# NVlabs/CenterPose

Measured on NVIDIA H100. Metric: images/sec at 512x512 DLA-34 (dla_34 + DCNv2, 7 heads, decode + PnP), higher is better.
Workload: dtype tf32x3

## Files before the change

### centerpose_b200/_lib.py

```python
import ctypes
import os

HERE = os.path.dirname(os.path.abspath(__file__))
LIB_PATH = os.environ.get("CP_LIB_PATH") or os.path.join(HERE, "libcenterpose_b200.so")

CP_MAX_HEADS = 16
CP_POSE_RECORD = 192
CP_DETS_RECORD = 128
CP_META_DOUBLES = 16
CP_MAX_K = 128
CP_MAX_MODELS = 16

CP_ARCH_DLA34 = 0
CP_ARCH_DLAV1_34 = 1
CP_ARCH_RES_18, CP_ARCH_RES_34, CP_ARCH_RES_50, CP_ARCH_RES_101, CP_ARCH_RES_152 = 2, 3, 4, 5, 6
CP_PREC_FP32 = 0
CP_PREC_TF32X3 = 1
CP_PREC_BF16 = 2
CP_PREC_TF32 = 3
PRECISIONS = {"fp32": CP_PREC_FP32, "tf32x3": CP_PREC_TF32X3, "bf16": CP_PREC_BF16, "tf32": CP_PREC_TF32}

P_SCORE, P_CLS, P_STATUS, P_NPTS, P_BBOX, P_CT, P_KPS = 0, 1, 2, 3, 4, 8, 10
P_KPS_DISP_MEAN, P_KPS_HM_MEAN, P_KPS_HM_STD, P_KPS_HM_HEIGHT, P_KPS_DISP_STD = 26, 42, 58, 74, 82
P_OBJ_SCALE, P_OBJ_SCALE_UNC, P_TRACKING, P_TRACKING_HP = 98, 101, 104, 106
# ... 39 lines not shown
FAM_NONE, FAM_IGEMM_FP32, FAM_STEM, FAM_CONV3_C16, FAM_IGEMM_UMMA, FAM_CONV_TMA, FAM_DCN_TMA = 0, 1, 2, 3, 4, 5, 6
FAM_MAXPOOL, FAM_UPADD, FAM_GN_RELU, FAM_GRU = 7, 8, 9, 10
FAMILY_NAMES = {FAM_NONE: "fused", FAM_IGEMM_FP32: "igemm_fp32", FAM_STEM: "stem", FAM_CONV3_C16: "conv3_c16",
                FAM_IGEMM_UMMA: "igemm_umma", FAM_CONV_TMA: "conv_tma", FAM_DCN_TMA: "dcn_tma", FAM_MAXPOOL: "maxpool",
                FAM_UPADD: "upadd", FAM_GN_RELU: "gn_relu", FAM_GRU: "gru"}


class CpOpStat(ctypes.Structure):
    _fields_ = [("name", ctypes.c_char * 96), ("kind", ctypes.c_int32), ("ms", ctypes.c_float),
                ("flops", ctypes.c_double), ("bytes", ctypes.c_double)]


class CpActDesc(ctypes.Structure):
    _fields_ = [("off", ctypes.c_int64), ("ext", ctypes.c_int32), ("C", ctypes.c_int32), ("H", ctypes.c_int32),
                ("W", ctypes.c_int32), ("stride", ctypes.c_int32)]


class CpOpDesc(ctypes.Structure):
    _fields_ = ([("name", ctypes.c_char * 96)] +
                [(n, ctypes.c_int32) for n in ("kind", "family", "x3", "nsrc")] +
                [("src", CpActDesc * 4), ("out", CpActDesc), ("out_head", ctypes.c_int32)] +
                [(n, ctypes.c_int32) for n in ("kh", "stride", "pad", "Cin", "Cout", "CoutPad", "Kpad")] +
                [("w", ctypes.c_void_p), ("w_ld", ctypes.c_int32), ("bias", ctypes.c_void_p)] +
                [(n, ctypes.c_int32) for n in ("relu", "has_res", "res_after_relu")] +
                [("res", CpActDesc), ("om", CpActDesc), ("up_w", ctypes.c_void_p), ("f", ctypes.c_int32),
                 ("has_skip", ctypes.c_int32), ("skip", CpActDesc), ("gamma", ctypes.c_void_p),
                 ("beta", ctypes.c_void_p), ("groups", ctypes.c_int32), ("gx", CpActDesc), ("gh", CpActDesc),
                 ("gprev", CpActDesc), ("first_step", ctypes.c_int32)] +
                [(n, ctypes.c_int32) for n in ("fuse_heads", "fused_away", "parent", "n_children")] +
                [("children", ctypes.c_int32 * CP_MAX_HEADS)])


class CpOpLaunch(ctypes.Structure):
    _fields_ = [(n, ctypes.c_int32) for n in ("family", "BN", "ksplit", "grid")]


class CpMemoryInfo(ctypes.Structure):
    _fields_ = [(n, ctypes.c_int64) for n in ("activation_bytes", "weight_bytes", "tile_bytes", "workspace_bytes")]


class CpActAlloc(ctypes.Structure):
    _fields_ = [("floats", ctypes.c_int64), ("off", ctypes.c_int64), ("first", ctypes.c_int32), ("last", ctypes.c_int32)]


class CpConfig(ctypes.Structure):
    _fields_ = [
        ("arch", ctypes.c_int32), ("tracking", ctypes.c_int32), ("tracking_task_gru", ctypes.c_int32),
        ("max_batch", ctypes.c_int32), ("height", ctypes.c_int32), ("width", ctypes.c_int32),
        ("precision", ctypes.c_int32), ("device", ctypes.c_int32), ("head_conv", ctypes.c_int32),
        ("num_heads", ctypes.c_int32),
        ("head_names", ctypes.c_char_p * CP_MAX_HEADS),
        ("head_channels", ctypes.c_int32 * CP_MAX_HEADS),
    ]


class CpHeads(ctypes.Structure):
    _fields_ = [(n, ctypes.c_void_p) for n in (
        "hm", "wh", "hps", "reg", "hm_hp", "hp_offset", "scale", "hps_uncertainty",
        "scale_uncertainty", "tracking", "tracking_hp")]


class CpDecodeParams(ctypes.Structure):
    _fields_ = [
        ("batch", ctypes.c_int32), ("out_h", ctypes.c_int32), ("out_w", ctypes.c_int32),
        ("num_classes", ctypes.c_int32), ("num_joints", ctypes.c_int32), ("K", ctypes.c_int32),
        ("rep_mode", ctypes.c_int32), ("use_moments", ctypes.c_int32), ("nms", ctypes.c_int32),
        ("visible_thresh", ctypes.c_int32), ("opencv_return", ctypes.c_int32),
# ... 126 lines not shown
```

### centerpose_b200/csrc/common.cuh

```cuda
#pragma once
#include <cuda_runtime.h>
#include <stdint.h>
#include <stdio.h>
#include <string>

#include "../../include/centerpose_b200.h"

namespace cp {

void set_error(const std::string& msg);
int fail(int code, const std::string& msg);
extern thread_local long long g_launch_counter;

#define CP_CUDA_CHECK(expr)                                                              \
  do {                                                                                   \
    cudaError_t _e = (expr);                                                             \
    if (_e != cudaSuccess)                                                               \
      return ::cp::fail(CP_ERR_CUDA, std::string(#expr) + ": " + cudaGetErrorString(_e)); \
  } while (0)

#define CP_LAUNCH_CHECK(what)                                                            \
  do {                                                                                   \
    cudaError_t _e = cudaGetLastError();                                                 \
    if (_e != cudaSuccess)                                                               \
// ... 25 lines not shown
  int resStride;
  int relu;
  int res_after_relu;
  float* out;
  int outStride;
  int out_nchw;
  const float* offmask;
  int omStride;
  int mask_is_logit;
  int mode;
  const void* wgt_umma;
  float* splitk_ws;
  size_t splitk_ws_floats;
  int fuse_n, fuse_hidden;
  const float* fuse_w[16];
  const float* fuse_b[16];
  float* fuse_out[16];
  int fuse_cout[16];
  int ipm;
  long long wstride, tstride;
  unsigned nchw_per_model;
};
inline int model_ipm(const IgemmParams& p) { return p.ipm > 0 ? p.ipm : p.B; }

int launch_igemm_fp32(const IgemmParams& p, cudaStream_t stream);

int decode_pnp_models(const cp_decode_params* prm, int models, const cp_heads* heads, const double* meta, float* dets,
                      float* poses, int32_t* n_valid, void* workspace, size_t workspace_bytes, void* stream);

struct LaunchInfo {
  int BN = 0;
  int ksplit = 1;
  long long grid = 0;
};

bool conv3_c16_supported(const IgemmParams& p);
int launch_conv3_c16(const IgemmParams& p, cudaStream_t stream);
bool stem_supported(const IgemmParams& p);
int launch_stem_conv(const IgemmParams& p, cudaStream_t s);

struct ConvKernel {
  int family = CP_FAM_IGEMM_FP32;
  bool x3 = false;
  bool round_out = false;
  int BN = 0;
  int cslab = 0;
  size_t wbytes = 0;
};
struct ConvPolicy {
  bool small_on_cuda_cores;
  bool dcn_tma;
  bool round_out;
  bool cuda_core_fallback;
};
inline bool known_precision(int32_t precision) {
  return precision == CP_PREC_FP32 || precision == CP_PREC_TF32X3 || precision == CP_PREC_BF16 || precision == CP_PREC_TF32;
}
inline bool gather_x3(int32_t precision) { return precision == CP_PREC_TF32 || precision == CP_PREC_TF32X3; }
ConvKernel select_conv_kernel(const IgemmParams& p, int32_t precision, const ConvPolicy& pol);
struct alignas(64) TmaMaps {
  unsigned char map[4][128];
};
int conv_encode(const ConvKernel& k, const IgemmParams& p, int Bmax, TmaMaps* maps);
int conv_pack(const ConvKernel& k, const IgemmParams& p, int ld, void* tiles, cudaStream_t s);
int conv_launch(const ConvKernel& k, const IgemmParams& p, const TmaMaps* maps, cudaStream_t s, LaunchInfo* info = nullptr);
int run_conv(IgemmParams& p, int32_t precision, const ConvPolicy& pol, cudaStream_t s);
// ... 101 lines not shown
```

### centerpose_b200/csrc/dcn_tma.cu

```cuda
#include <cuda.h>

#include "common.cuh"
#include "umma_common.cuh"

namespace cp {
namespace {

using namespace umma;

constexpr int DT_BM = 128;
constexpr int DT_THREADS = 512;
constexpr int DT_CS = 16;
constexpr int DT_PH = 8, DT_PW = 16;
constexpr int DT_HALO = 8;
constexpr int DT_SH = DT_PH + 2 * DT_HALO, DT_SW = DT_PW + 2 * DT_HALO;
constexpr uint32_t DT_SLAB_BYTES = DT_SH * DT_SW * DT_CS * 4;
constexpr uint32_t DT_COEF_BYTES = DT_BM * 9 * 16;

struct DcnTmaParams {
  CUtensorMap amap;
  const float* src;
  int srcStride;
  const float* offmask;
  int omStride, mask_is_logit;
  int B, H, W, Cin, Cout, CoutPad, BN;
  int tiles_x, tiles_per_image;
  long long total_tiles;
  int SB;
  int group;
  int AH;
  const float* bias;
  const float* residual;
  int resStride, relu, res_after_relu;
  float* out;
  int outStride, out_nchw, round_tf32;
  const unsigned char* wtiles;
  int ksplit, sps;
  float* part;
  int ipm;
  long long wstride, tstride;
};

struct DcnCtl {
  unsigned long long s_full[2], s_empty[2];
  unsigned long long a_full[2], a_empty[2];
  unsigned long long c_full[2], c_empty[2];
  unsigned long long b_full[8], b_empty[8];
};

constexpr int RB_DX = 14, RB_DY = 15, RB_W = 16, RB_SLAB = 20, RB_LIVE = 21;

__device__ __forceinline__ void coef_row(const DcnTmaParams& p, const float* __restrict__ om, int oy, int ox, int ys,
                                         int xs, uint32_t dst) {
  float o[27];
#pragma unroll
  for (int j = 0; j < 27; ++j) o[j] = __ldg(om + j);
  const int H = p.H, W = p.W;
#pragma unroll
  for (int tap = 0; tap < 9; ++tap) {
    const int ky = tap / 3, kx = tap - ky * 3;
    float mm = o[18 + tap];
    if (p.mask_is_logit) mm = 1.0f / (1.0f + expf(-mm));
    const float h_im = (float)(oy - 1 + ky) + o[2 * tap], w_im = (float)(ox - 1 + kx) + o[2 * tap + 1];
    float lh = 0.f, lw = 0.f, mk = 0.f;
    uint32_t pk = 0;
    if (h_im > -1.f && w_im > -1.f && h_im < (float)H && w_im < (float)W) {
      const int h_low = (int)floorf(h_im), w_low = (int)floorf(w_im);
      lh = h_im - (float)h_low;
      lw = w_im - (float)w_low;
      const bool t_ok = h_low >= 0, b_ok = h_low + 1 <= H - 1, l_ok = w_low >= 0, r_ok = w_low + 1 <= W - 1;
      const int hl = t_ok ? h_low : 0, hb = b_ok ? h_low + 1 : H - 1;
      const int wl = l_ok ? w_low : 0, wr = r_ok ? w_low + 1 : W - 1;
      const bool in_slab = (hl >= ys) && (hb < ys + DT_SH) && (wl >= xs) && (wr < xs + DT_SW);
      pk = in_slab ? (uint32_t)((hl - ys) * DT_SW + (wl - xs)) : (uint32_t)((hl << 7) | wl);
      pk |= (uint32_t)(wr - wl) << RB_DX;
      pk |= (uint32_t)(hb - hl) << RB_DY;
      pk |= (uint32_t)((t_ok && l_ok) ? 1 : 0) << (RB_W + 0);
      pk |= (uint32_t)((t_ok && r_ok) ? 1 : 0) << (RB_W + 1);
// ... 162 lines not shown
            }
#pragma unroll
            for (int c = 0; c < 4; ++c) {
              c3[c] = ld_shared_v4f(b3 ^ ((uint32_t)c << 4));
              c4[c] = ld_shared_v4f(b4 ^ ((uint32_t)c << 4));
            }
#pragma unroll
            for (int c = 0; c < 4; ++c) {
              v[c].x = w1 * c1[c].x + w2 * c2[c].x + w3 * c3[c].x + w4 * c4[c].x;
              v[c].y = w1 * c1[c].y + w2 * c2[c].y + w3 * c3[c].y + w4 * c4[c].y;
              v[c].z = w1 * c1[c].z + w2 * c2[c].z + w3 * c3[c].z + w4 * c4[c].z;
              v[c].w = w1 * c1[c].w + w2 * c2[c].w + w3 * c3[c].w + w4 * c4[c].w;
            }
          } else {
            const int hl = (int)((pk >> 7) & 127u), wl = (int)(pk & 127u);
            const float* g = gimg + ((size_t)hl * p.W + wl) * p.srcStride + (s0 + s) * DT_CS;
            const size_t dx = (size_t)((pk >> RB_DX) & 1u) * p.srcStride;
            const size_t dy = (size_t)((pk >> RB_DY) & 1u) * p.W * p.srcStride;
#pragma unroll
            for (int c = 0; c < 4; ++c) {
              const float4 c1 = __ldg(reinterpret_cast<const float4*>(g) + c);
              const float4 c2 = __ldg(reinterpret_cast<const float4*>(g + dx) + c);
              const float4 c3 = __ldg(reinterpret_cast<const float4*>(g + dy) + c);
              const float4 c4 = __ldg(reinterpret_cast<const float4*>(g + dy + dx) + c);
              v[c].x = w1 * c1.x + w2 * c2.x + w3 * c3.x + w4 * c4.x;
              v[c].y = w1 * c1.y + w2 * c2.y + w3 * c3.y + w4 * c4.y;
              v[c].z = w1 * c1.z + w2 * c2.z + w3 * c3.z + w4 * c4.z;
              v[c].w = w1 * c1.w + w2 * c2.w + w3 * c3.w + w4 * c4.w;
            }
          }
        }
        const int sa = (int)(cnt & (uint32_t)(p.AH - 1));
        const uint32_t a_dst = a_row + (uint32_t)sa * a_stage + (asw << 4);
        mbar_wait(smem_u32(&ctl->a_empty[sa]), ((cnt >> (p.AH - 1)) & 1u) ^ 1u);
#pragma unroll
        for (int c = 0; c < 4; ++c) {
          const uint32_t off = (uint32_t)c << 4;
          if (X3)
            st_shared_v4f(a_dst ^ off, v[c].x, v[c].y, v[c].z, v[c].w);
          else
            st_shared_v4f(a_dst ^ off, tf32_round(v[c].x), tf32_round(v[c].y), tf32_round(v[c].z), tf32_round(v[c].w));
        }
        fence_proxy_async_smem();
        __syncwarp();
        if (lane == 0) mbar_arrive(smem_u32(&ctl->a_full[sa]));
        ++cnt;
      }
      __syncwarp();
      if (lane == 0) {
        mbar_arrive(smem_u32(&ctl->s_empty[ss]));
        mbar_arrive(smem_u32(&ctl->c_empty[cb]));
      }
      if (++ss == 2) {
        ss = 0;
        ps ^= 1u;
      }
      if (++cb == 2) {
        cb = 0;
        pc ^= 1u;
      }
    }
  } else {
    asm volatile("setmaxnreg.inc.sync.aligned.u32 176;");
    const int c = warp >= 12 ? 1 : 0, wt = tid & 127;
    float* dstage = reinterpret_cast<float*>(smem + (drain0 - sbase)) + (size_t)c * (DRAIN_STAGE_BYTES / 4);
    EpiParams ep;
    ep.bias = p.bias;
// ... 2 lines not shown
    ep.relu = p.relu;
    ep.res_after_relu = p.res_after_relu;
    ep.round_tf32 = p.round_tf32;
    ep.out = p.out;
    ep.outStride = p.outStride;
    ep.out_nchw = p.out_nchw;
    ep.Cout = p.Cout;
    ep.CoutPad = p.CoutPad;
    ep.H = p.H;
    ep.W = p.W;
    int cb = 0;
    uint32_t pc = 0;
    auto make_records = [&](long long t) {
      const long long mt = (t / KS_SPLIT) / n_tiles;
      const int im = (int)(mt / p.tiles_per_image);
      const int pt = (int)(mt - (long long)im * p.tiles_per_image);
      const int y0 = (pt / p.tiles_x) * DT_PH, x0 = (pt % p.tiles_x) * DT_PW;
      const int oy = y0 + (wt >> 4), ox = x0 + (wt & 15);
      mbar_wait(smem_u32(&ctl->c_empty[cb]), pc ^ 1u);
      coef_row(p, p.offmask + ((size_t)((size_t)im * p.H + oy) * p.W + ox) * p.omStride, oy, ox, y0 - DT_HALO, x0 - DT_HALO,
               coef0 + (uint32_t)cb * DT_COEF_BYTES + (uint32_t)wt * 144u);
      __syncwarp();
      if (lane == 0) mbar_arrive(smem_u32(&ctl->c_full[cb]));
      if (++cb == 2) {
        cb = 0;
        pc ^= 1u;
      }
    };
    if (c == 0 && (long long)blockIdx.x < total_tiles) make_records(blockIdx.x);
    const uint32_t bar_a_full = smem_u32(&ctl->a_full[0]), bar_a_empty = smem_u32(&ctl->a_empty[0]);
    const uint32_t bar_b_full = smem_u32(&ctl->b_full[0]), bar_b_empty = smem_u32(&ctl->b_empty[0]);
    int sb = 0;
    uint32_t pb = 0, cnt = 0;
    float acc[BN / 2];
    float sums[X3 ? BN / 2 : 1];
#pragma unroll
    for (int j = 0; j < BN / 2; ++j) acc[j] = 0.f;
    for (long long tile = blockIdx.x; tile < total_tiles; tile += gridDim.x) {
      if (c == 0 && tile + gridDim.x < total_tiles) make_records(tile + gridDim.x);
#pragma unroll
      for (int j = 0; j < (X3 ? BN / 2 : 1); ++j) sums[j] = 0.f;
      int gk = 0;
      for (int kbi = 0; kbi < KB; ++kbi, ++cnt) {
        const uint32_t sa = cnt & (uint32_t)(p.AH - 1);
        mbar_wait(bar_a_full + 8u * sa, (cnt >> (p.AH - 1)) & 1u);
        mbar_wait(bar_b_full + 8u * (uint32_t)sb, pb);
        const uint32_t a_tile = atiles0 + sa * a_stage + (uint32_t)c * 64u * 64u;
        const uint64_t db = make_desc(btiles0 + (uint32_t)sb * btile_bytes, DT_CS);
        if (X3)
          mma_kblock_x3<BN, 2>(acc, a_tile, wt, db, ((uint32_t)BN * 64u) >> 4, gk == 0);
        else
          mma_kblock<BN, false, false, 2>(acc, make_desc(a_tile, DT_CS), db, 0, 0, kbi == 0);
        if (wt == 0) {
          mbar_arrive(bar_a_empty + 8u * sa);
          mbar_arrive(bar_b_empty + 8u * (uint32_t)sb);
        }
        if (++sb == p.SB) {
          sb = 0;
          pb ^= 1u;
        }
        if (X3) {
          if (gk == p.group - 1 || kbi == KB - 1) {
#pragma unroll
            for (int j = 0; j < (X3 ? BN / 2 : 1); ++j) sums[j] += acc[X3 ? j : 0];
            gk = 0;
          } else {
            ++gk;
          }
        }
      }
      const int n_tile = (int)((tile / KS_SPLIT) % n_tiles);
      const long long m_tile = (tile / KS_SPLIT) / n_tiles;
      const int n = (int)(m_tile / p.tiles_per_image);
      const int pt = (int)(m_tile - (long long)n * p.tiles_per_image);
      const int col_end = min(p.Cout, (n_tile + 1) * BN);
      if (MULTI) ep.bias = p.bias + (size_t)(n / p.ipm) * p.wstride;
      auto fn = [&](int r, int cb0, float (&v)[16]) {
        if (cb0 >= BN) return;
        const int i = c * 64 + r;
        if (KS_SPLIT > 1) {
          float4* part_row = reinterpret_cast<float4*>(p.part) + ((size_t)tile * (BN >> 2) + (cb0 >> 2)) * 128 + i;
#pragma unroll
          for (int q = 0; q < 4; ++q) __stcg(part_row + (size_t)q * 128, make_float4(v[4 * q], v[4 * q + 1], v[4 * q + 2], v[4 * q + 3]));
        } else {
          const int oy = (pt / p.tiles_x) * DT_PH + (i >> 4), ox = (pt % p.tiles_x) * DT_PW + (i & 15);
          const int m = (n * p.H + oy) * p.W + ox;
          epilogue_row<16>(ep, v, true, m, n, oy, ox, n_tile * BN + cb0, col_end);
        }
      };
      if constexpr (X3)
        drain_rows<BN>(sums, dstage, wt, 1 + c, fn);
      else
        drain_rows<BN>(acc, dstage, wt, 1 + c, fn);
    }
  }
}

template <bool MULTI>
__global__ void __launch_bounds__(256) dcn_tma_splitk_finish(const __grid_constant__ DcnTmaParams p, long long mn_tiles) {
  splitk_finish<MULTI>(p, DT_BM, mn_tiles, [&](long long mn, int i, int* n, int* oy, int* ox) {
    const long long m_tile = mn / (p.CoutPad / p.BN);
// ... 18 lines not shown
  return dcn_tma_tile_n(p.CoutPad, x3) != 0;
}

int dcn_tma_encode(const IgemmParams& p, int Bmax, void* map_out) {
  return tma_encode_nhwc_box(p.src[0], p.srcC[0], p.Win, p.Hin, Bmax, p.srcStride[0], DT_CS, DT_SW, DT_SH, 1, map_out);
}

int launch_dcn_tma(const IgemmParams& p, const void* map, const ConvKernel& k, cudaStream_t stream, LaunchInfo* info) {
  const bool x3 = k.x3;
  if (!p.wgt_umma) return fail(CP_ERR_INVALID, "dcn_tma: weight tiles missing");
  if (!dcn_tma_supported(p, x3)) return fail(CP_ERR_INVALID, "dcn_tma: unsupported shape");
  DcnTmaParams q;
  memset(&q, 0, sizeof(q));
  memcpy(&q.amap, map, sizeof(CUtensorMap));
  q.src = p.src[0];
  q.srcStride = p.srcStride[0];
  q.offmask = p.offmask;
  q.omStride = p.omStride;
  q.mask_is_logit = p.mask_is_logit;
  q.B = p.B;
  q.H = p.Hin;
  q.W = p.Win;
  q.Cin = p.Cin;
  q.Cout = p.Cout;
  q.CoutPad = p.CoutPad;
  q.BN = k.BN;
  q.tiles_x = p.Win / DT_PW;
  q.tiles_per_image = q.tiles_x * (p.Hin / DT_PH);
  const long long mn = (long long)q.tiles_per_image * p.B * (p.CoutPad / q.BN);
  const uint32_t a_stage = 8192u;
  q.group = kX3GroupBlocks * 2;
  const uint32_t btile = (uint32_t)q.BN * 64u * (x3 ? 2u : 1u);
  const size_t budget = 226 * 1024;
  q.AH = 2;
  size_t fixed = 1024 + 2 * (size_t)DT_COEF_BYTES + 1024 + 2 * (size_t)DT_SLAB_BYTES + (size_t)q.AH * a_stage +
                 2 * (size_t)DRAIN_STAGE_BYTES;
  if (fixed + 3 * (size_t)btile > budget) {
    q.AH = 1;
    fixed -= a_stage;
  }
  if (fixed + 2 * (size_t)btile > budget) return fail(CP_ERR_INVALID, "dcn_tma: tile does not fit shared memory");
  q.SB = (int)((budget - fixed) / btile);
  if (q.SB > 8) q.SB = 8;
  q.bias = p.bias;
  q.residual = p.residual;
  q.resStride = p.resStride;
  q.relu = p.relu;
  q.res_after_relu = p.res_after_relu;
  q.out = p.out;
  q.outStride = p.outStride;
  q.out_nchw = p.out_nchw;
  q.round_tf32 = k.round_out;
  q.wtiles = (const unsigned char*)p.wgt_umma;
  q.ipm = model_ipm(p);
  q.wstride = p.wstride;
  q.tstride = p.tstride;
  const bool multi = p.B > q.ipm;
  const size_t smem = fixed + (size_t)q.SB * btile;
  void (*kern)(DcnTmaParams) = nullptr;
  switch (q.BN) {
    case 16: kern = multi ? (x3 ? dcn_tma_kernel<true, 16, true> : dcn_tma_kernel<false, 16, true>)
                          : (x3 ? dcn_tma_kernel<true, 16, false> : dcn_tma_kernel<false, 16, false>); break;
    case 32: kern = multi ? (x3 ? dcn_tma_kernel<true, 32, true> : dcn_tma_kernel<false, 32, true>)
                          : (x3 ? dcn_tma_kernel<true, 32, false> : dcn_tma_kernel<false, 32, false>); break;
    case 64: kern = multi ? (x3 ? dcn_tma_kernel<true, 64, true> : dcn_tma_kernel<false, 64, true>)
                          : (x3 ? dcn_tma_kernel<true, 64, false> : dcn_tma_kernel<false, 64, false>); break;
    case 128: kern = multi ? (x3 ? dcn_tma_kernel<true, 128, true> : dcn_tma_kernel<false, 128, true>)
                           : (x3 ? dcn_tma_kernel<true, 128, false> : dcn_tma_kernel<false, 128, false>); break;
    default: return fail(CP_ERR_INVALID, "dcn_tma: unsupported N tile");
  }
  static PerDevice<bool, 16> configured;
  const int slot = (multi ? 8 : 0) + (x3 ? 4 : 0) + (q.BN == 128 ? 3 : (q.BN == 64 ? 2 : (q.BN == 32 ? 1 : 0)));
  if (!configured.here(slot)) {
    CP_CUDA_CHECK(cudaFuncSetAttribute(kern, cudaFuncAttributeMaxDynamicSharedMemorySize, 227 * 1024));
    configured.here(slot) = true;
  }
  int num_sms = 0;
  if (int rc = device_sm_count(&num_sms)) return rc;
  const int nslab = p.Cin / DT_CS;
  q.part = p.splitk_ws;
  q.ksplit = splitk_factor(mn, nslab, num_sms, (size_t)DT_BM * q.BN, p.splitk_ws_floats);
  q.sps = nslab / q.ksplit;
  q.total_tiles = mn * q.ksplit;
  const unsigned grid = (unsigned)(q.total_tiles < num_sms ? q.total_tiles : num_sms);
  CP_CUDA_CHECK(launch_kernel(kern, dim3(grid), dim3(DT_THREADS), smem, stream, q));
  CP_LAUNCH_CHECK("dcn_tma_kernel");
  if (info) {
    info->BN = q.BN;
    info->ksplit = q.ksplit;
    info->grid = grid;
  }
  if (q.ksplit > 1) {
    const long long threads = mn * (q.BN / 4) * DT_BM;
    CP_CUDA_CHECK(launch_kernel(multi ? dcn_tma_splitk_finish<true> : dcn_tma_splitk_finish<false>, dim3((unsigned)((threads + 255) / 256)), dim3(256), 0, stream, q, mn));
    CP_LAUNCH_CHECK("dcn_tma_splitk_finish");
  }
  return CP_OK;
}

}
```

### centerpose_b200/csrc/plan.cu

```cuda
#include <stdlib.h>
#include <string.h>

#include <map>
#include <memory>
#include <set>
#include <string>
#include <vector>

#include "arena_pack.h"
#include "common.cuh"

namespace cp {

thread_local std::string g_last_error;
void set_error(const std::string& msg) { g_last_error = msg; }
thread_local long long g_launch_counter = 0;
thread_local int g_pdl = 0;

int fail(int code, const std::string& msg) {
  g_last_error = msg;
  return code;
}

namespace {
// ... 962 lines not shown
static bool pdl_wanted(long long pixels) {
  if (getenv("CP_NO_PDL")) return false;
  if (const char* e = getenv("CP_PDL")) return atoi(e) != 0;
  return pixels <= 8ll * 512 * 512;
}

static int run_op(cp_plan* P, size_t idx, int batch, const float* const ext[4], float* const* head_out, cudaStream_t s,
                  cp_op_launch* info) {
  int rc;
  const Op& op = P->ops[idx];
  const int images = batch * P->models;
  const long long wstride = (long long)P->w_floats;
  cp_op_launch li{};
  li.ksplit = 1;
  if (op.fused_away) {
    if (info) *info = li;
    return CP_OK;
  }
  switch (op.type) {
    case OP_IGEMM: {
      for (int i = 0; i < op.nsrc; ++i)
        if (op.src[i].ext >= 0 && !ext[op.src[i].ext]) return fail(CP_ERR_INVALID, "cp_forward: a tracking input tensor is null");
      IgemmParams p;
      igemm_params(P, op, batch, ext, head_out, &p);
      p.wgt_umma = P->umma_wts + op.tile_off;
      p.splitk_ws = P->splitk_ws;
      p.splitk_ws_floats = P->splitk_ws ? kSplitkWsFloats : 0;
      LaunchInfo tc;
      li.family = op.kernel.family;
      if ((rc = conv_launch(op.kernel, p, &op.maps, s, &tc))) return rc;
      li.BN = tc.BN;
      li.ksplit = tc.ksplit;
      li.grid = (int32_t)tc.grid;
      break;
    }
    case OP_MAXPOOL:
      li.family = CP_FAM_MAXPOOL;
      if ((rc = launch_maxpool2(P->act + op.src[0].off, P->act + op.out.off, images, op.src[0].H, op.src[0].W,
                                op.src[0].C, s)))
        return rc;
      break;
    case OP_MAXPOOL3:
      li.family = CP_FAM_MAXPOOL;
      if ((rc = launch_maxpool3s2(P->act + op.src[0].off, op.has_res ? P->act + op.res.off : nullptr, P->act + op.out.off,
                                  images, op.src[0].H, op.src[0].W, op.src[0].C, s)))
        return rc;
      break;
    case OP_UPADD:
      li.family = CP_FAM_UPADD;
      if ((rc = launch_upsample_add(P->act + op.src[0].off, P->wts + op.upw_off,
                                    op.has_skip ? P->act + op.skip.off : nullptr, P->act + op.out.off, images,
                                    op.src[0].H, op.src[0].W, op.src[0].C, op.f, s, batch, wstride)))
        return rc;
      break;
    case OP_GN_RELU:
      li.family = CP_FAM_GN_RELU;
      if ((rc = launch_group_norm_relu(P->act + op.out.off, P->wts + op.gamma_off, P->wts + op.beta_off, images,
                                       op.out.H * op.out.W, op.out.C, op.out.stride, 0, op.groups, 1e-5f,
                                       P->gn_stats, s, batch, wstride)))
        return rc;
      break;
    case OP_GRU:
      li.family = CP_FAM_GRU;
      if ((rc = launch_gru_gates(P->act + op.gx.off, op.first_step ? nullptr : P->act + op.gh.off,
                                 op.first_step ? nullptr : P->act + op.gprev.off, P->act + op.out.off,
                                 images * op.out.H * op.out.W, op.out.C, op.first_step, s)))
// ... 329 lines not shown
```

### centerpose_b200/csrc/umma_common.cuh

```cuda
#pragma once
#include <cuda.h>
#include <cuda_runtime.h>
#include <stdint.h>
#include <stdio.h>

namespace cp {
namespace umma {

__device__ __forceinline__ uint32_t smem_u32(const void* p) { return (uint32_t)__cvta_generic_to_shared(p); }

__device__ __forceinline__ void mbar_init(uint32_t bar, uint32_t count) {
  asm volatile("mbarrier.init.shared::cta.b64 [%0], %1;" ::"r"(bar), "r"(count));
}
__device__ __forceinline__ void mbar_arrive(uint32_t bar) {
  asm volatile("mbarrier.arrive.shared::cta.b64 _, [%0];" ::"r"(bar) : "memory");
}
__device__ __forceinline__ void mbar_arrive_expect_tx(uint32_t bar, uint32_t bytes) {
  asm volatile("mbarrier.arrive.expect_tx.shared::cta.b64 _, [%0], %1;" ::"r"(bar), "r"(bytes) : "memory");
}
__device__ __forceinline__ bool mbar_try_wait(uint32_t bar, uint32_t parity) {
  uint32_t ok;
  asm volatile(
      "{\n\t.reg .pred p;\n\tmbarrier.try_wait.parity.shared::cta.b64 p, [%1], %2;\n\tselp.b32 %0, 1, 0, p;\n\t}"
      : "=r"(ok)
// ... 141 lines not shown
  for (int ks = 0; ks < KS; ++ks) {
    const uint32_t sd = (fresh && ks == 0) ? 0u : 1u;
    if (X3) {
      wgmma_tf32<BN>(acc, da + a_lo + 2u * ks, db + 2u * ks, sd);
      wgmma_tf32<BN>(acc, da + 2u * ks, db + b_lo + 2u * ks, 1u);
    } else if (BF16) {
      wgmma_bf16<BN>(acc, da + 2u * ks, db + 2u * ks, sd);
    } else {
      wgmma_tf32<BN>(acc, da + 2u * ks, db + 2u * ks, sd);
    }
  }
  if (X3) {
#pragma unroll
    for (int ks = 0; ks < KS; ++ks) wgmma_tf32<BN>(acc, da + 2u * ks, db + 2u * ks, 1u);
  }
  wg_commit();
}
template <int BN, bool X3, bool BF16, int KS>
__device__ __forceinline__ void mma_kblock(float (&acc)[BN / 2], uint64_t da, uint64_t db, uint32_t a_lo, uint32_t b_lo,
                                           bool fresh) {
  mma_kblock_issue<BN, X3, BF16, KS>(acc, da, db, a_lo, b_lo, fresh);
  wg_wait<0>();
}

__device__ __forceinline__ float tf32_round(float x) {
  return __uint_as_float((__float_as_uint(x) + 0x1000u) & 0xffffe000u);
}
__device__ __forceinline__ void ldsm_x4(uint32_t (&r)[4], uint32_t addr) {
  asm volatile("ldmatrix.sync.aligned.m8n8.x4.shared.b16 {%0, %1, %2, %3}, [%4];"
               : "=r"(r[0]), "=r"(r[1]), "=r"(r[2]), "=r"(r[3])
               : "r"(addr));
}

template <int BN, int KS>
__device__ __forceinline__ void mma_kblock_x3(float (&acc)[BN / 2], uint32_t a_tile, int wt, uint64_t db, uint32_t b_lo,
                                              bool fresh) {
  const uint32_t lane = (uint32_t)wt & 31u;
  const uint32_t row = (uint32_t)(wt >> 5) * 16u + (lane & 7u) + ((lane >> 3) & 1u) * 8u;
  const uint32_t a_row = a_tile + row * (32u * KS);
  const uint32_t x = ((lane >> 4) << 4) ^ ((a_row >> 3) & (KS == 4 ? 0x70u : 0x30u));
  uint32_t hi[KS][4], lo[KS][4];
#pragma unroll
  for (int ks = 0; ks < KS; ++ks) {
    ldsm_x4(hi[ks], a_row + (((uint32_t)ks << 5) ^ x));
#pragma unroll
    for (int j = 0; j < 4; ++j) {
      const float v = __uint_as_float(hi[ks][j]);
      const float h = tf32_round(v);
      lo[ks][j] = __float_as_uint(tf32_round(v - h));
      hi[ks][j] = __float_as_uint(h);
    }
  }
  wg_fence();
#pragma unroll
  for (int ks = 0; ks < KS; ++ks) {
    wgmma_tf32_rs<BN>(acc, lo[ks], db + 2u * ks, (fresh && ks == 0) ? 0u : 1u);
    wgmma_tf32_rs<BN>(acc, hi[ks], db + b_lo + 2u * ks, 1u);
  }
#pragma unroll
  for (int ks = 0; ks < KS; ++ks) wgmma_tf32_rs<BN>(acc, hi[ks], db + 2u * ks, 1u);
  wg_commit();
  wg_wait<0>();
#pragma unroll
  for (int ks = 0; ks < KS; ++ks)
#pragma unroll
    for (int j = 0; j < 4; ++j) asm volatile("" : "+r"(hi[ks][j]), "+r"(lo[ks][j]));
}

__device__ __forceinline__ uint32_t pack_bf16x2(float a, float b) {
  uint32_t r;
  asm("cvt.rn.bf16x2.f32 %0, %1, %2;" : "=r"(r) : "f"(b), "f"(a));
  return r;
}
__device__ __forceinline__ void st_shared_v4(uint32_t addr, uint32_t a, uint32_t b, uint32_t c, uint32_t d) {
  asm volatile("st.shared.v4.b32 [%0], {%1, %2, %3, %4};" ::"r"(addr), "r"(a), "r"(b), "r"(c), "r"(d) : "memory");
}
__device__ __forceinline__ void st_shared_v4f(uint32_t addr, float a, float b, float c, float d) {
  asm volatile("st.shared.v4.f32 [%0], {%1, %2, %3, %4};" ::"r"(addr), "f"(a), "f"(b), "f"(c), "f"(d) : "memory");
}
__device__ __forceinline__ float4 ld_shared_v4f(uint32_t addr) {
  float4 v;
  asm volatile("ld.shared.v4.f32 {%0,%1,%2,%3}, [%4];" : "=f"(v.x), "=f"(v.y), "=f"(v.z), "=f"(v.w) : "r"(addr) : "memory");
  return v;
}

__device__ __forceinline__ void tma_load_4d(uint32_t dst, const CUtensorMap* map, int c0, int c1, int c2, int c3, uint32_t bar) {
  asm volatile(
      "cp.async.bulk.tensor.4d.shared::cluster.global.tile.mbarrier::complete_tx::bytes [%0], [%1, {%2, %3, %4, %5}], [%6];" ::"r"(dst),
      "l"(map), "r"(c0), "r"(c1), "r"(c2), "r"(c3), "r"(bar)
      : "memory");
}
__device__ __forceinline__ void tma_load_2d(uint32_t dst, const CUtensorMap* map, int c0, int c1, uint32_t bar) {
  asm volatile("cp.async.bulk.tensor.2d.shared::cluster.global.tile.mbarrier::complete_tx::bytes [%0], [%1, {%2, %3}], [%4];" ::"r"(dst),
               "l"(map), "r"(c0), "r"(c1), "r"(bar)
               : "memory");
}
__device__ __forceinline__ bool elect_one() {
  uint32_t pred;
  asm volatile("{\n\t.reg .pred p;\n\telect.sync _|p, 0xffffffff;\n\tselp.u32 %0, 1, 0, p;\n\t}" : "=r"(pred));
// ... 127 lines not shown
```

### centerpose_b200/engine.py

```python
import ctypes

import numpy as np
import torch

from . import _lib

HEAD_FIELDS = ("hm", "wh", "hps", "reg", "hm_hp", "hp_offset", "scale", "hps_uncertainty",
               "scale_uncertainty", "tracking", "tracking_hp")
_VISIBLE = {"book": 6, "chair": 6, "cereal_box": 6, "camera": 3, "bottle": 3, "cup": 3,
            "bike": 0, "laptop": 0, "shoe": 0}


def _ptr(t):
    return ctypes.c_void_p(t.data_ptr()) if t is not None else ctypes.c_void_p(0)


def _stream():
    return ctypes.c_void_p(torch.cuda.current_stream().cuda_stream)


def decode_params(opt=None, **over):
    g = lambda n, d: over.get(n, getattr(opt, n, d) if opt is not None else d)
    p = _lib.CpDecodeParams()
    p.num_classes = int(g("num_classes", 1))
# ... 266 lines not shown
                v = getattr(d, name)
                if isinstance(v, _lib.CpActDesc):
                    v = self._act(v)
                elif name == "src":
                    v = [self._act(a) for a in v][:max(1, int(d.nsrc))]
                elif name == "children":
                    v = [int(c) for c in v][:int(d.n_children)]
                elif name == "name":
                    v = v.decode()
                elif v is None:
                    v = 0
                r[name] = v
            r["index"] = i
            out.append(r)
        return out

    def arena(self):
        p, n = ctypes.c_void_p(), ctypes.c_int64()
        _lib.check(self.L.cp_plan_arena(self.plan, ctypes.byref(p), ctypes.byref(n)), "cp_plan_arena")
        return _device_view(p.value, int(n.value), self.device)

    def run_ops(self, x, first, last, out, pre_img=None, pre_hm=None, pre_hm_hp=None):
        B, xs = self._check_inputs(x, pre_img, pre_hm, pre_hm_hp)
        for n, c in self.heads.items():
            self._out_tensor(out[n], "out[%s]" % n, self._head_shape(B, c), torch.float32)
        hp = (ctypes.c_void_p * len(self.head_names))(*[out[n].data_ptr() for n in self.head_names])
        n = max(0, last - first)
        info = (_lib.CpOpLaunch * max(1, n))()
        with torch.cuda.device(self.device):
            rc = self.L.cp_plan_run_ops(self.plan, B, first, last, _ptr(xs[0]), _ptr(xs[1]), _ptr(xs[2]), _ptr(xs[3]),
                                        hp, _stream(), info)
        _lib.check(rc, "cp_plan_run_ops")
        return [dict(family=int(info[i].family), BN=int(info[i].BN), ksplit=int(info[i].ksplit),
                     grid=int(info[i].grid)) for i in range(n)]

    def infer(self, x, meta, prm, pre_img=None, pre_hm=None, pre_hm_hp=None, heads_out=None, want_dets=False,
              poses=None, n_valid=None, dets=None):
        B, xs = self._check_inputs(x, pre_img, pre_hm, pre_hm_hp)
        lead = self._lead(B)
        if not torch.is_tensor(meta) or tuple(meta.shape) != (B, _lib.CP_META_DOUBLES):
            raise ValueError("meta must be a [%d,%d] tensor (make_meta)" % (B, _lib.CP_META_DOUBLES))
        if meta.device != self.device or meta.dtype != torch.float64 or not meta.is_contiguous():
            meta = meta.to(self.device, torch.float64).contiguous()
        if self.models > 1:
            prms = list(prm)
            if len(prms) != self.models:
                raise ValueError("a plan of %d models needs %d decode parameter sets, got %d" % (self.models, self.models,
                                                                                                len(prms)))
            K = prms[0].K
        else:
            K = prm.K
        if poses is None:
            poses = torch.empty(lead + (K, _lib.CP_POSE_RECORD), dtype=torch.float32, device=self.device)
        else:
            self._out_tensor(poses, "poses", lead + (K, _lib.CP_POSE_RECORD), torch.float32)
        if n_valid is None:
            n_valid = torch.empty(lead, dtype=torch.int32, device=self.device)
        else:
            self._out_tensor(n_valid, "n_valid", lead, torch.int32)
        if want_dets and dets is None:
            dets = torch.empty(lead + (K, _lib.CP_DETS_RECORD), dtype=torch.float32, device=self.device)
        elif dets is not None:
            self._out_tensor(dets, "dets", lead + (K, _lib.CP_DETS_RECORD), torch.float32)
        hp = None
        if heads_out is not None:
            for n, c in self.heads.items():
                self._out_tensor(heads_out[n], "heads_out[%s]" % n, self._head_shape(B, c), torch.float32)
# ... 277 lines not shown
```

### include/centerpose_b200.h

```cpp
#ifndef CENTERPOSE_B200_H_
#define CENTERPOSE_B200_H_

#include <stddef.h>
#include <stdint.h>

#ifdef __cplusplus
extern "C" {
#endif

#define CP_ABI_VERSION 1

enum cp_status {
  CP_OK = 0,
  CP_ERR_INVALID = -1,
  CP_ERR_CUDA = -2,
  CP_ERR_NOT_LOADED = -3,
  CP_ERR_MISSING_KEY = -4,
  CP_ERR_SHAPE = -5
};

enum cp_arch {
  CP_ARCH_DLA34 = 0,
  CP_ARCH_DLAV1_34 = 1,
  CP_ARCH_RES_18 = 2,
// ... 100 lines not shown
  int32_t kind;
  int32_t family;
  int32_t x3;
  int32_t nsrc;
  cp_act_desc src[4];
  cp_act_desc out;
  int32_t out_head;
  int32_t kh, stride, pad, Cin, Cout, CoutPad, Kpad;
  const float* w;
  int32_t w_ld;
  const float* bias;
  int32_t relu, has_res, res_after_relu;
  cp_act_desc res;
  cp_act_desc om;
  const float* up_w;
  int32_t f, has_skip;
  cp_act_desc skip;
  const float* gamma;
  const float* beta;
  int32_t groups;
  cp_act_desc gx, gh, gprev;
  int32_t first_step;
  int32_t fuse_heads;
  int32_t fused_away;
  int32_t parent;
  int32_t n_children;
  int32_t children[CP_MAX_HEADS];
} cp_op_desc;
typedef struct cp_op_launch {
  int32_t family;
  int32_t BN;
  int32_t ksplit;
  int32_t grid;
} cp_op_launch;
int cp_plan_op_desc(const cp_plan* plan, int32_t i, cp_op_desc* out);
int cp_plan_op_desc_model(const cp_plan* plan, int32_t model, int32_t i, cp_op_desc* out);
int cp_plan_arena(const cp_plan* plan, float** act, int64_t* floats);
int cp_plan_run_ops(cp_plan* plan, int32_t batch, int32_t first, int32_t last, const float* images, const float* pre_img,
                    const float* pre_hm, const float* pre_hm_hp, float* const* head_out, void* stream,
                    cp_op_launch* info);

int64_t cp_plan_bytes(const cp_plan* plan);
int32_t cp_plan_forward_launches(const cp_plan* plan);

typedef struct cp_heads {
  const float* hm;
  const float* wh;
  const float* hps;
  const float* reg;
  const float* hm_hp;
  const float* hp_offset;
  const float* scale;
  const float* hps_uncertainty;
  const float* scale_uncertainty;
  const float* tracking;
  const float* tracking_hp;
} cp_heads;

typedef struct cp_decode_params {
  int32_t batch, out_h, out_w;
  int32_t num_classes;
  int32_t num_joints;
  int32_t K;
  int32_t rep_mode;
  int32_t use_moments;
  int32_t nms;
// ... 227 lines not shown
```

Measured before the change: 763.8.

## Deepen DCN A-tile ring and overlap TF32x3 wgmma kblocks in flight

After: 772.3, median of 6. 1.1% higher.

```diff
diff --git a/centerpose_b200/_lib.py b/centerpose_b200/_lib.py
--- a/centerpose_b200/_lib.py
+++ b/centerpose_b200/_lib.py
@@ -95,7 +95,7 @@
 
 
 class CpOpLaunch(ctypes.Structure):
-    _fields_ = [(n, ctypes.c_int32) for n in ("family", "BN", "ksplit", "grid")]
+    _fields_ = [(n, ctypes.c_int32) for n in ("family", "BN", "ksplit", "grid", "a_stages")]
 
 
 class CpMemoryInfo(ctypes.Structure):
diff --git a/centerpose_b200/csrc/common.cuh b/centerpose_b200/csrc/common.cuh
--- a/centerpose_b200/csrc/common.cuh
+++ b/centerpose_b200/csrc/common.cuh
@@ -81,6 +81,7 @@
   int BN = 0;
   int ksplit = 1;
   long long grid = 0;
+  int a_stages = 0;
 };
 
 bool conv3_c16_supported(const IgemmParams& p);
diff --git a/centerpose_b200/csrc/dcn_tma.cu b/centerpose_b200/csrc/dcn_tma.cu
--- a/centerpose_b200/csrc/dcn_tma.cu
+++ b/centerpose_b200/csrc/dcn_tma.cu
@@ -29,6 +29,7 @@
   int SB;
   int group;
   int AH;
+  int ah_shift;
   const float* bias;
   const float* residual;
   int resStride, relu, res_after_relu;
@@ -43,7 +44,7 @@
 
 struct DcnCtl {
   unsigned long long s_full[2], s_empty[2];
-  unsigned long long a_full[2], a_empty[2];
+  unsigned long long a_full[4], a_empty[4];
   unsigned long long c_full[2], c_empty[2];
   unsigned long long b_full[8], b_empty[8];
 };
@@ -272,7 +273,7 @@
         }
         const int sa = (int)(cnt & (uint32_t)(p.AH - 1));
         const uint32_t a_dst = a_row + (uint32_t)sa * a_stage + (asw << 4);
-        mbar_wait(smem_u32(&ctl->a_empty[sa]), ((cnt >> (p.AH - 1)) & 1u) ^ 1u);
+        mbar_wait(smem_u32(&ctl->a_empty[sa]), ((cnt >> p.ah_shift) & 1u) ^ 1u);
 #pragma unroll
         for (int c = 0; c < 4; ++c) {
           const uint32_t off = (uint32_t)c << 4;
@@ -341,41 +342,77 @@
     const uint32_t bar_b_full = smem_u32(&ctl->b_full[0]), bar_b_empty = smem_u32(&ctl->b_empty[0]);
     int sb = 0;
     uint32_t pb = 0, cnt = 0;
+    auto acquire = [&](uint32_t& a_tile, uint64_t& db) {
+      const uint32_t sa = cnt & (uint32_t)(p.AH - 1);
+      mbar_wait(bar_a_full + 8u * sa, (cnt >> p.ah_shift) & 1u);
+      mbar_wait(bar_b_full + 8u * (uint32_t)sb, pb);
+      a_tile = atiles0 + sa * a_stage + (uint32_t)c * 64u * 64u;
+      db = make_desc(btiles0 + (uint32_t)sb * btile_bytes, DT_CS);
+      ++cnt;
+      if (++sb == p.SB) {
+        sb = 0;
+        pb ^= 1u;
+      }
+    };
+    auto release = [&](int back) {
+      if (wt == 0) {
+        const int s = sb - back;
+        mbar_arrive(bar_a_empty + 8u * ((cnt - (uint32_t)back) & (uint32_t)(p.AH - 1)));
+        mbar_arrive(bar_b_empty + 8u * (uint32_t)(s < 0 ? s + p.SB : s));
+      }
+    };
     float acc[BN / 2];
     float sums[X3 ? BN / 2 : 1];
+    X3Frag<2> f0, f1;
 #pragma unroll
     for (int j = 0; j < BN / 2; ++j) acc[j] = 0.f;
     for (long long tile = blockIdx.x; tile < total_tiles; tile += gridDim.x) {
       if (c == 0 && tile + gridDim.x < total_tiles) make_records(tile + gridDim.x);
-#pragma unroll
-      for (int j = 0; j < (X3 ? BN / 2 : 1); ++j) sums[j] = 0.f;
-      int gk = 0;
-      for (int kbi = 0; kbi < KB; ++kbi, ++cnt) {
-        const uint32_t sa = cnt & (uint32_t)(p.AH - 1);
-        mbar_wait(bar_a_full + 8u * sa, (cnt >> (p.AH - 1)) & 1u);
-        mbar_wait(bar_b_full + 8u * (uint32_t)sb, pb);
-        const uint32_t a_tile = atiles0 + sa * a_stage + (uint32_t)c * 64u * 64u;
-        const uint64_t db = make_desc(btiles0 + (uint32_t)sb * btile_bytes, DT_CS);
-        if (X3)
-          mma_kblock_x3<BN, 2>(acc, a_tile, wt, db, ((uint32_t)BN * 64u) >> 4, gk == 0);
-        else
+      uint32_t a_tile;
+      uint64_t db;
+      if constexpr (X3) {
+#pragma unroll
+        for (int j = 0; j < BN / 2; ++j) sums[j] = 0.f;
+        for (int kb0 = 0; kb0 < KB; kb0 += p.group) {
+          const int n_kb = min(p.group, KB - kb0);
+          if constexpr (BN > 64) {
+            for (int i = 0; i < n_kb; ++i) {
+              acquire(a_tile, db);
+              mma_kblock_x3<BN, 2>(acc, a_tile, wt, db, ((uint32_t)BN * 64u) >> 4, i == 0);
+              release(1);
+            }
+          } else {
+            for (int i = 0; i < n_kb; i += 2) {
+              acquire(a_tile, db);
+              mma_kblock_x3_issue<BN, 2>(acc, f0, a_tile, wt, db, ((uint32_t)BN * 64u) >> 4, i == 0);
+              if (i > 0) {
+                wg_wait<1>();
+                x3_frag_hold(f1);
+                release(2);
+              }
+              if (i + 1 < n_kb) {
+                acquire(a_tile, db);
+                mma_kblock_x3_issue<BN, 2>(acc, f1, a_tile, wt, db, ((uint32_t)BN * 64u) >> 4, false);
+                wg_wait<1>();
+                x3_frag_hold(f0);
+                release(2);
+              }
+            }
+            wg_wait<0>();
+            x3_frag_hold(f0);
+            x3_frag_hold(f1);
+            release(1);
+          }
+#pragma unroll
+          for (int j = 0; j < BN / 2; ++j) sums[j] += acc[j];
+        }
+#pragma unroll
+        for (int j = 0; j < BN / 2; ++j) acc[j] = 0.f;
+      } else {
+        for (int kbi = 0; kbi < KB; ++kbi) {
+          acquire(a_tile, db);
           mma_kblock<BN, false, false, 2>(acc, make_desc(a_tile, DT_CS), db, 0, 0, kbi == 0);
-        if (wt == 0) {
-          mbar_arrive(bar_a_empty + 8u * sa);
-          mbar_arrive(bar_b_empty + 8u * (uint32_t)sb);
-        }
-        if (++sb == p.SB) {
-          sb = 0;
-          pb ^= 1u;
-        }
-        if (X3) {
-          if (gk == p.group - 1 || kbi == KB - 1) {
-#pragma unroll
-            for (int j = 0; j < (X3 ? BN / 2 : 1); ++j) sums[j] += acc[X3 ? j : 0];
-            gk = 0;
-          } else {
-            ++gk;
-          }
+          release(1);
         }
       }
       const int n_tile = (int)((tile / KS_SPLIT) % n_tiles);
@@ -460,13 +497,11 @@
   q.group = kX3GroupBlocks * 2;
   const uint32_t btile = (uint32_t)q.BN * 64u * (x3 ? 2u : 1u);
   const size_t budget = 226 * 1024;
-  q.AH = 2;
-  size_t fixed = 1024 + 2 * (size_t)DT_COEF_BYTES + 1024 + 2 * (size_t)DT_SLAB_BYTES + (size_t)q.AH * a_stage +
-                 2 * (size_t)DRAIN_STAGE_BYTES;
-  if (fixed + 3 * (size_t)btile > budget) {
-    q.AH = 1;
-    fixed -= a_stage;
-  }
+  const size_t base = 1024 + 2 * (size_t)DT_COEF_BYTES + 1024 + 2 * (size_t)DT_SLAB_BYTES + 2 * (size_t)DRAIN_STAGE_BYTES;
+  q.AH = 4;
+  while (q.AH > 1 && base + (size_t)q.AH * a_stage + 3 * (size_t)btile > budget) q.AH >>= 1;
+  q.ah_shift = q.AH == 4 ? 2 : q.AH - 1;
+  const size_t fixed = base + (size_t)q.AH * a_stage;
   if (fixed + 2 * (size_t)btile > budget) return fail(CP_ERR_INVALID, "dcn_tma: tile does not fit shared memory");
   q.SB = (int)((budget - fixed) / btile);
   if (q.SB > 8) q.SB = 8;
@@ -517,6 +552,7 @@
     info->BN = q.BN;
     info->ksplit = q.ksplit;
     info->grid = grid;
+    info->a_stages = q.AH;
   }
   if (q.ksplit > 1) {
     const long long threads = mn * (q.BN / 4) * DT_BM;
diff --git a/centerpose_b200/csrc/plan.cu b/centerpose_b200/csrc/plan.cu
--- a/centerpose_b200/csrc/plan.cu
+++ b/centerpose_b200/csrc/plan.cu
@@ -1018,6 +1018,7 @@
       li.BN = tc.BN;
       li.ksplit = tc.ksplit;
       li.grid = (int32_t)tc.grid;
+      li.a_stages = tc.a_stages;
       break;
     }
     case OP_MAXPOOL:
diff --git a/centerpose_b200/csrc/umma_common.cuh b/centerpose_b200/csrc/umma_common.cuh
--- a/centerpose_b200/csrc/umma_common.cuh
+++ b/centerpose_b200/csrc/umma_common.cuh
@@ -197,39 +197,52 @@
                : "r"(addr));
 }
 
+template <int KS>
+struct X3Frag {
+  uint32_t hi[KS][4], lo[KS][4];
+};
 template <int BN, int KS>
-__device__ __forceinline__ void mma_kblock_x3(float (&acc)[BN / 2], uint32_t a_tile, int wt, uint64_t db, uint32_t b_lo,
-                                              bool fresh) {
+__device__ __forceinline__ void mma_kblock_x3_issue(float (&acc)[BN / 2], X3Frag<KS>& f, uint32_t a_tile, int wt,
+                                                    uint64_t db, uint32_t b_lo, bool fresh) {
   const uint32_t lane = (uint32_t)wt & 31u;
   const uint32_t row = (uint32_t)(wt >> 5) * 16u + (lane & 7u) + ((lane >> 3) & 1u) * 8u;
   const uint32_t a_row = a_tile + row * (32u * KS);
   const uint32_t x = ((lane >> 4) << 4) ^ ((a_row >> 3) & (KS == 4 ? 0x70u : 0x30u));
-  uint32_t hi[KS][4], lo[KS][4];
 #pragma unroll
   for (int ks = 0; ks < KS; ++ks) {
-    ldsm_x4(hi[ks], a_row + (((uint32_t)ks << 5) ^ x));
+    ldsm_x4(f.hi[ks], a_row + (((uint32_t)ks << 5) ^ x));
 #pragma unroll
     for (int j = 0; j < 4; ++j) {
-      const float v = __uint_as_float(hi[ks][j]);
+      const float v = __uint_as_float(f.hi[ks][j]);
       const float h = tf32_round(v);
-      lo[ks][j] = __float_as_uint(tf32_round(v - h));
-      hi[ks][j] = __float_as_uint(h);
+      f.lo[ks][j] = __float_as_uint(tf32_round(v - h));
+      f.hi[ks][j] = __float_as_uint(h);
     }
   }
   wg_fence();
 #pragma unroll
   for (int ks = 0; ks < KS; ++ks) {
-    wgmma_tf32_rs<BN>(acc, lo[ks], db + 2u * ks, (fresh && ks == 0) ? 0u : 1u);
-    wgmma_tf32_rs<BN>(acc, hi[ks], db + b_lo + 2u * ks, 1u);
-  }
-#pragma unroll
-  for (int ks = 0; ks < KS; ++ks) wgmma_tf32_rs<BN>(acc, hi[ks], db + 2u * ks, 1u);
+    wgmma_tf32_rs<BN>(acc, f.lo[ks], db + 2u * ks, (fresh && ks == 0) ? 0u : 1u);
+    wgmma_tf32_rs<BN>(acc, f.hi[ks], db + b_lo + 2u * ks, 1u);
+  }
+#pragma unroll
+  for (int ks = 0; ks < KS; ++ks) wgmma_tf32_rs<BN>(acc, f.hi[ks], db + 2u * ks, 1u);
   wg_commit();
+}
+template <int KS>
+__device__ __forceinline__ void x3_frag_hold(X3Frag<KS>& f) {
+#pragma unroll
+  for (int ks = 0; ks < KS; ++ks)
+#pragma unroll
+    for (int j = 0; j < 4; ++j) asm volatile("" : "+r"(f.hi[ks][j]), "+r"(f.lo[ks][j]));
+}
+template <int BN, int KS>
+__device__ __forceinline__ void mma_kblock_x3(float (&acc)[BN / 2], uint32_t a_tile, int wt, uint64_t db, uint32_t b_lo,
+                                              bool fresh) {
+  X3Frag<KS> f;
+  mma_kblock_x3_issue<BN, KS>(acc, f, a_tile, wt, db, b_lo, fresh);
   wg_wait<0>();
-#pragma unroll
-  for (int ks = 0; ks < KS; ++ks)
-#pragma unroll
-    for (int j = 0; j < 4; ++j) asm volatile("" : "+r"(hi[ks][j]), "+r"(lo[ks][j]));
+  x3_frag_hold(f);
 }
 
 __device__ __forceinline__ uint32_t pack_bf16x2(float a, float b) {
diff --git a/centerpose_b200/engine.py b/centerpose_b200/engine.py
--- a/centerpose_b200/engine.py
+++ b/centerpose_b200/engine.py
@@ -322,7 +322,7 @@
                                         hp, _stream(), info)
         _lib.check(rc, "cp_plan_run_ops")
         return [dict(family=int(info[i].family), BN=int(info[i].BN), ksplit=int(info[i].ksplit),
-                     grid=int(info[i].grid)) for i in range(n)]
+                     grid=int(info[i].grid), a_stages=int(info[i].a_stages)) for i in range(n)]
 
     def infer(self, x, meta, prm, pre_img=None, pre_hm=None, pre_hm_hp=None, heads_out=None, want_dets=False,
               poses=None, n_valid=None, dets=None):
diff --git a/include/centerpose_b200.h b/include/centerpose_b200.h
--- a/include/centerpose_b200.h
+++ b/include/centerpose_b200.h
@@ -156,6 +156,7 @@
   int32_t BN;
   int32_t ksplit;
   int32_t grid;
+  int32_t a_stages;
 } cp_op_launch;
 int cp_plan_op_desc(const cp_plan* plan, int32_t i, cp_op_desc* out);
 int cp_plan_op_desc_model(const cp_plan* plan, int32_t model, int32_t i, cp_op_desc* out);
```
